# Microsoft/multiverso

Measured on AMD Instinct MI355X. Metric: MatrixTable Add+Get updates/sec (whole node), higher is better.
Workload: dtype fp32; 1 GPU; model=MatrixTable 1000000x128 dense sgd updater, global_batch=1, parallelism=ps-sharded dp1 (reduce-scatter/all-gather over xGMI)

## Files before the change

multiverso_amd/ops/csrc/bindings.cpp:

```cpp

#include <torch/extension.h>
#include <ATen/hip/HIPContext.h>
#include <cstdint>

extern "C" {
void mv_launch_copy(void*, const float*, int, int64_t, hipStream_t);
void mv_launch_add(float*, const void*, int, int64_t, hipStream_t, int);
void mv_launch_add_f64(double*, const double*, int64_t, hipStream_t, int);
void mv_launch_add_i32(int32_t*, const int32_t*, int64_t, hipStream_t, int);
void mv_launch_add_i64(int64_t*, const int64_t*, int64_t, hipStream_t, int);
void mv_launch_sgd(float*, const void*, void*, int, float, int64_t,
                   hipStream_t, int);
void mv_launch_sgd_f64(double*, const double*, double*, double, int64_t,
                       hipStream_t, int);
void mv_launch_momentum(float*, float*, const void*, void*, int, float,
                        int64_t, hipStream_t, int);
void mv_launch_momentum_f64(double*, double*, const double*, double, int64_t,
                            hipStream_t, int);
void mv_launch_adagrad(float*, float*, const void*, void*, int, float, float,
                       float, int64_t, hipStream_t, int);
void mv_launch_adagrad_f64(double*, double*, const double*, double, double,
                           double, int64_t, hipStream_t, int);
void mv_launch_dcasgd(float*, float*, const void*, void*, int, float, float,
                      int64_t, hipStream_t, int);
void mv_launch_dcasgda(float*, float*, float*, const void*, void*, int, float,
                       float, float, float, int64_t, hipStream_t, int);
void mv_launch_adam(float*, float*, float*, const void*, void*, int, double,
                    double, double, double, double, double, int64_t,
                    hipStream_t, int);
void mv_launch_adam_f64(double*, double*, double*, const double*, double,
                        double, double, double, double, double, int64_t,
                        hipStream_t, int);
void mv_launch_onebit_encode(const float*, float*, uint8_t*, int64_t,
                             hipStream_t);
void mv_launch_onebit_decode_sum(float*, const uint8_t*, int, int64_t,
                                 hipStream_t);
void mv_launch_row_gather(void*, int, const float*, const int64_t*, int64_t,
                          int64_t, hipStream_t);
void mv_launch_row_scatter_add(float*, const void*, int, const int64_t*, float,
                               int64_t, int64_t, int, hipStream_t);
void mv_launch_w2v(float*, float*, float*, float*, const int64_t*, const int*,
                   const int64_t*, const float*, const int*, float, int64_t,
                   int64_t, int, int, hipStream_t);
void mv_launch_w2v_ns(float*, float*, float*, float*, const int64_t*,
                      const int*, const int64_t*, const int64_t*, int64_t,
                      int, uint64_t, float, int64_t, int64_t, int, int,
                      hipStream_t);
void mv_launch_lr_sigmoid_fwd(const float*, const int64_t*, const float*,
                              const int*, const float*, const float*,
                              float*, float*, int64_t, hipStream_t);
void mv_launch_lr_sigmoid_scatter(float*, const int64_t*, const float*,
                                  const int*, const float*, float, int,
                                  float, int64_t, hipStream_t);
void mv_launch_row_scatter_adagrad(float*, float*, const void*, int,
                                   const int64_t*, float, float, float,
                                   int64_t, int64_t, int, hipStream_t);
void mv_launch_row_momentum(float*, float*, const void*, int, const int64_t*,
                            const int64_t*, float, int64_t, int64_t,
                            hipStream_t);
void mv_launch_row_dcasgd(float*, float*, const void*, int, const int64_t*,
                          const int64_t*, float, float, int64_t, int64_t,
                          hipStream_t);
void mv_launch_row_dcasgda(float*, float*, float*, const void*, int,
                           const int64_t*, const int64_t*, float, float,
                           float, float, int64_t, int64_t, hipStream_t);
void mv_launch_row_adam(float*, float*, float*, const void*, int,
                        const int64_t*, const int64_t*, double, double,
                        double, double, double, double, int64_t, int64_t,
                        hipStream_t);
void mv_launch_lr_softmax_fwd(const float*, const int64_t*, const float*,
                              const int*, const float*, const float*,
                              float*, float*, int64_t, int64_t, hipStream_t);
void mv_launch_lr_softmax_scatter(float*, const int64_t*, const float*,
                                  const int*, const float*, float, int,
                                  float, int64_t, int64_t, hipStream_t);
void mv_launch_lr_dense_post(float*, const float*, const float*, float*,
                             float, int64_t, int64_t, hipStream_t);
int mv_launch_lr_dense_fwd(const float*, const float*, const float*,
                           const float*, float*, float*, float, int64_t,
                           int64_t, int64_t, int, hipStream_t);
void mv_launch_lr_ftrl_fwd(const float*, const int64_t*, const float*,
                           const int*, const float*, const float*, float*,
                           float*, float, float, float, float, int64_t,
                           int64_t, hipStream_t);
void mv_launch_lr_ftrl_scatter(float*, const int64_t*, const float*,
                               const int*, const float*, float, float,
                               float, float, int64_t, int64_t, hipStream_t);
}

namespace {

hipStream_t cur_stream() {
  return at::hip::getCurrentHIPStream().stream();
}

void check_f32(const torch::Tensor& t, const char* name) {
  TORCH_CHECK(t.is_cuda(), name, " must be on GPU");
  TORCH_CHECK(t.is_contiguous(), name, " must be contiguous");
  TORCH_CHECK(t.scalar_type() == torch::kFloat32, name, " must be fp32");
}

void check_dev(const torch::Tensor& t, const char* name,
               torch::ScalarType st) {
  TORCH_CHECK(t.is_cuda(), name, " must be on GPU");
  TORCH_CHECK(t.is_contiguous(), name, " must be contiguous");
  TORCH_CHECK(t.scalar_type() == st, name, " dtype mismatch");
}

using Named = std::pair<const char*, torch::Tensor>;
int64_t check_same(std::initializer_list<Named> ts,
                   c10::optional<torch::ScalarType> st = c10::nullopt) {
  for (const auto& t : ts) {
    if (st) check_dev(t.second, t.first, *st);
    else check_f32(t.second, t.first);
  }
  int64_t n = ts.begin()->second.numel();
  for (const auto& t : ts)
    TORCH_CHECK(t.second.numel() == n, "size mismatch");
  return n;
}

float* f32(const torch::Tensor& t) { return t.data_ptr<float>(); }
double* f64(const torch::Tensor& t) { return t.data_ptr<double>(); }

constexpr int kWireDelta = 1, kWireOut = 2;

int wire_bit(const torch::Tensor& t, const char* name, int64_t n, int bit,
             c10::optional<torch::ScalarType> st = c10::nullopt) {
  TORCH_CHECK(t.is_cuda(), name, " must be on GPU");
  TORCH_CHECK(t.is_contiguous(), name, " must be contiguous");
  TORCH_CHECK(t.numel() == n, "size mismatch");
  auto want = st.value_or(torch::kFloat32);
  if (want == torch::kFloat32 && t.scalar_type() == torch::kBFloat16)
    return bit;
  if (st) {
    TORCH_CHECK(t.scalar_type() == want, name, " dtype mismatch");
  } else {
    TORCH_CHECK(t.scalar_type() == want, name, " must be fp32 or bf16");
  }
  return 0;
}

void nt_copy(torch::Tensor dst, torch::Tensor src) {
  int64_t n = check_same({{"src", src}});
  int wire = wire_bit(dst, "dst", n, kWireOut);
  mv_launch_copy(dst.data_ptr(), f32(src), wire, n, cur_stream());
}

void add_inplace(torch::Tensor data, torch::Tensor delta, bool reverse) {
  auto st = data.scalar_type();
  int64_t n = check_same({{"data", data}}, st);
  int wire = wire_bit(delta, "delta", n, kWireDelta, st);
  if (st == torch::kFloat32)
    mv_launch_add(f32(data), delta.data_ptr(), wire, n, cur_stream(), reverse);
  else if (st == torch::kFloat64)
    mv_launch_add_f64(f64(data), f64(delta), n, cur_stream(), reverse);
  else if (st == torch::kInt32)
    mv_launch_add_i32(data.data_ptr<int32_t>(), delta.data_ptr<int32_t>(), n,
// ... 420 lines not shown
  TORCH_CHECK(ptr.scalar_type() == torch::kInt32, "ptr must be int32");
  int64_t B = ptr.numel() - 1;
  TORCH_CHECK(err.numel() == B, "err size mismatch");
  mv_launch_lr_sigmoid_scatter(w.data_ptr<float>(), keys.data_ptr<int64_t>(),
                               vals.data_ptr<float>(), ptr.data_ptr<int>(),
                               err.data_ptr<float>(), (float)lr,
                               (int)reg_type, (float)reg_coef, B,
                               cur_stream());
}

void lr_softmax_forward(torch::Tensor w, torch::Tensor keys,
                        torch::Tensor vals, torch::Tensor ptr,
                        torch::Tensor labels,
                        c10::optional<torch::Tensor> wts,
                        torch::Tensor err, torch::Tensor loss, int64_t K) {
  check_f32(w, "w"); check_f32(vals, "vals"); check_f32(labels, "labels");
  check_f32(err, "err"); check_f32(loss, "loss");
  TORCH_CHECK(keys.scalar_type() == torch::kInt64, "keys must be int64");
  TORCH_CHECK(ptr.scalar_type() == torch::kInt32, "ptr must be int32");
  TORCH_CHECK(K >= 2 && K <= 64,
              "fused softmax supports 2..64 classes (got ", K, ")");
  int64_t B = ptr.numel() - 1;
  TORCH_CHECK(labels.numel() == B && loss.numel() == B, "batch mismatch");
  TORCH_CHECK(err.numel() == B * K, "err must be [B, K]");
  TORCH_CHECK(keys.numel() == vals.numel(), "keys/vals mismatch");
  const float* wp = nullptr;
  if (wts.has_value()) {
    check_f32(*wts, "wts");
    TORCH_CHECK(wts->numel() == B, "weights size mismatch");
    wp = wts->data_ptr<float>();
  }
  mv_launch_lr_softmax_fwd(w.data_ptr<float>(), keys.data_ptr<int64_t>(),
                           vals.data_ptr<float>(), ptr.data_ptr<int>(),
                           labels.data_ptr<float>(), wp,
                           err.data_ptr<float>(), loss.data_ptr<float>(),
                           B, K, cur_stream());
}

void lr_softmax_scatter(torch::Tensor w, torch::Tensor keys,
                        torch::Tensor vals, torch::Tensor ptr,
                        torch::Tensor err, double lr, int64_t reg_type,
                        double reg_coef, int64_t K) {
  check_f32(w, "w"); check_f32(vals, "vals"); check_f32(err, "err");
  TORCH_CHECK(keys.scalar_type() == torch::kInt64, "keys must be int64");
  TORCH_CHECK(ptr.scalar_type() == torch::kInt32, "ptr must be int32");
  int64_t B = ptr.numel() - 1;
  TORCH_CHECK(err.numel() == B * K, "err must be [B, K]");
  mv_launch_lr_softmax_scatter(w.data_ptr<float>(), keys.data_ptr<int64_t>(),
                               vals.data_ptr<float>(), ptr.data_ptr<int>(),
                               err.data_ptr<float>(), (float)lr,
                               (int)reg_type, (float)reg_coef, B, K,
                               cur_stream());
}

void lr_ftrl_forward(torch::Tensor zn, torch::Tensor keys,
                     torch::Tensor vals, torch::Tensor ptr,
                     torch::Tensor labels, c10::optional<torch::Tensor> wts,
                     torch::Tensor err, torch::Tensor loss, double alpha,
                     double beta, double l1, double l2, int64_t K) {
  check_f32(zn, "zn"); check_f32(vals, "vals"); check_f32(labels, "labels");
  check_f32(err, "err"); check_f32(loss, "loss");
  TORCH_CHECK(keys.scalar_type() == torch::kInt64, "keys must be int64");
  TORCH_CHECK(ptr.scalar_type() == torch::kInt32, "ptr must be int32");
  TORCH_CHECK(K >= 1 && K <= 32,
              "fused FTRL supports 1..32 outputs (got ", K, ")");
  int64_t B = ptr.numel() - 1;
  TORCH_CHECK(labels.numel() == B && loss.numel() == B, "batch mismatch");
  TORCH_CHECK(err.numel() == B * K, "err must be [B, K]");
  const float* wp = nullptr;
  if (wts.has_value()) {
    check_f32(*wts, "wts");
    wp = wts->data_ptr<float>();
  }
  mv_launch_lr_ftrl_fwd(zn.data_ptr<float>(), keys.data_ptr<int64_t>(),
                        vals.data_ptr<float>(), ptr.data_ptr<int>(),
                        labels.data_ptr<float>(), wp, err.data_ptr<float>(),
                        loss.data_ptr<float>(), (float)(1.0 / alpha),
                        (float)beta, (float)l1, (float)l2, B, K,
                        cur_stream());
}

void lr_dense_post(torch::Tensor logits, torch::Tensor labels,
                   c10::optional<torch::Tensor> wts, torch::Tensor loss_acc,
                   double inv_b) {
  check_f32(logits, "logits"); check_f32(labels, "labels");
  check_f32(loss_acc, "loss_acc");
  int64_t B = labels.numel();
  TORCH_CHECK(B > 0 && logits.numel() % B == 0,
              "logits/labels batch mismatch");
  int64_t K = logits.numel() / B;
  TORCH_CHECK(K >= 1 && K <= 64,
              "fused dense post supports 1..64 classes (got ", K, ")");
  TORCH_CHECK(loss_acc.numel() == 1, "loss_acc must be a scalar");
  const float* wp = nullptr;
  if (wts.has_value()) {
    check_f32(*wts, "wts");
    TORCH_CHECK(wts->numel() == B, "weights size mismatch");
    wp = wts->data_ptr<float>();
  }
  mv_launch_lr_dense_post(logits.data_ptr<float>(),
                          labels.data_ptr<float>(), wp,
                          loss_acc.data_ptr<float>(), (float)inv_b, B, K,
                          cur_stream());
}

bool lr_dense_fwd(torch::Tensor x, torch::Tensor w, torch::Tensor labels,
                  c10::optional<torch::Tensor> wts, torch::Tensor diff,
                  torch::Tensor loss_acc, double inv_b, bool nt) {
  check_f32(x, "x"); check_f32(w, "w"); check_f32(labels, "labels");
  check_f32(diff, "diff"); check_f32(loss_acc, "loss_acc");
  TORCH_CHECK(x.dim() == 2 && w.dim() == 2 && x.size(1) == w.size(0),
              "x [B,d] and w [d,K] shape mismatch");
  TORCH_CHECK(x.is_contiguous() && w.is_contiguous(), "x/w must be "
              "contiguous");
  int64_t B = x.size(0), d = x.size(1), K = w.size(1);
  TORCH_CHECK(labels.numel() == B, "labels batch mismatch");
  TORCH_CHECK(diff.numel() == B * K, "diff must be [B, K]");
  TORCH_CHECK(loss_acc.numel() == 1, "loss_acc must be a scalar");
  const float* wp = nullptr;
  if (wts.has_value()) {
    check_f32(*wts, "wts");
    TORCH_CHECK(wts->numel() == B, "weights size mismatch");
    wp = wts->data_ptr<float>();
  }
  return mv_launch_lr_dense_fwd(
             x.data_ptr<float>(), w.data_ptr<float>(),
             labels.data_ptr<float>(), wp, diff.data_ptr<float>(),
             loss_acc.data_ptr<float>(), (float)inv_b, B, d, K,
             nt ? 1 : 0, cur_stream()) != 0;
}


void lr_ftrl_scatter(torch::Tensor zn, torch::Tensor keys,
                     torch::Tensor vals, torch::Tensor ptr,
                     torch::Tensor err, double alpha, double beta, double l1,
                     double l2, int64_t K) {
  check_f32(zn, "zn"); check_f32(vals, "vals"); check_f32(err, "err");
  TORCH_CHECK(keys.scalar_type() == torch::kInt64, "keys must be int64");
  TORCH_CHECK(ptr.scalar_type() == torch::kInt32, "ptr must be int32");
  int64_t B = ptr.numel() - 1;
  TORCH_CHECK(err.numel() == B * K, "err must be [B, K]");
  mv_launch_lr_ftrl_scatter(zn.data_ptr<float>(), keys.data_ptr<int64_t>(),
                            vals.data_ptr<float>(), ptr.data_ptr<int>(),
                            err.data_ptr<float>(), (float)(1.0 / alpha),
                            (float)beta, (float)l1, (float)l2, B, K,
                            cur_stream());
}

}

PYBIND11_MODULE(TORCH_EXTENSION_NAME, m) {
  auto rev = py::arg("reverse") = false;
  auto data = py::arg("data"), delta = py::arg("delta"), out = py::arg("out");
  m.def("add_inplace", &add_inplace, "K1: data += delta (fp32, fused)", data,
        delta, rev);
  m.def("nt_copy", &nt_copy,
        "K7: non-temporal streaming copy (a bf16 dst narrows)");
  m.def("sgd_update", &sgd_update, "K2: data -= delta", data, delta, rev);
  m.def("momentum_update", &momentum_update, "K3: fused momentum update",
        data, py::arg("m"), delta, py::arg("mu"), rev);
  m.def("adagrad_update", &adagrad_update, "K4: fused adagrad update", data,
        py::arg("gsq"), delta, py::arg("lr"), py::arg("rho"), py::arg("eps"),
        rev);
  m.def("momentum_copy_update", &momentum_copy_update,
        "fused momentum Add+Get", data, py::arg("m"), delta, out,
        py::arg("mu"), rev);
  m.def("adagrad_copy_update", &adagrad_copy_update,
        "fused adagrad Add+Get", data, py::arg("gsq"), delta, out,
        py::arg("lr"), py::arg("rho"), py::arg("eps"), rev);
  m.def("dcasgd_copy_update", &dcasgd_copy_update,
        "fused dcasgd Add+Get", data, py::arg("bak"), delta, out,
        py::arg("lr"), py::arg("lambda_"), rev);
  m.def("dcasgda_copy_update", &dcasgda_copy_update,
        "fused dcasgda Add+Get", data, py::arg("bak"), py::arg("msq"), delta,
        out, py::arg("lr"), py::arg("lambda_"), py::arg("rho"),
        py::arg("eps"), rev);
  m.def("sgd_copy_update", &sgd_copy_update,
        "fused Add+Get: data (+/-)= delta; out = data (saves the Get's "
        "shard re-read at N=1)", data, delta, out, py::arg("sign"), rev);
  m.def("dcasgd_update", &dcasgd_update,
        "DC-ASGD: delay-compensated update with per-worker backup", data,
        py::arg("bak"), delta, py::arg("lr"), py::arg("lambda_"), rev);
  m.def("dcasgda_update", &dcasgda_update,
        "DC-ASGD-a: adaptive lambda via mean-square of gradients", data,
        py::arg("bak"), py::arg("msq"), delta, py::arg("lr"),
        py::arg("lambda_"), py::arg("rho"), py::arg("eps"), rev);
  m.def("adam_update", &adam_update,
        "fused Adam/AdamW step (fp32, fp64); step = lr/(1-b1^t), "
        "rbc2 = 1/sqrt(1-b2^t), decay = 1-lr*wd",
        py::arg("data"), py::arg("m"), py::arg("v"), py::arg("delta"),
        py::arg("b1"), py::arg("b2"), py::arg("step"), py::arg("rbc2"),
        py::arg("decay"), py::arg("eps"), rev);
  m.def("adam_copy_update", &adam_copy_update, "fused adam Add+Get",
        py::arg("data"), py::arg("m"), py::arg("v"), py::arg("delta"),
        py::arg("out"), py::arg("b1"), py::arg("b2"), py::arg("step"),
        py::arg("rbc2"), py::arg("decay"), py::arg("eps"), rev);
  m.def("onebit_encode", &onebit_encode,
        "1-bit wire: payload = code(residual + delta), residual = the error",
        py::arg("delta"), py::arg("residual"), py::arg("payload"));
  m.def("onebit_decode_sum", &onebit_decode_sum,
        "1-bit wire: out = sum over nparts payloads of their decoded values",
        py::arg("out"), py::arg("payloads"), py::arg("nparts"));
  m.def("row_gather", &row_gather,
        "K6: out[i] = shard[rows[i]]; dtype=torch.bfloat16 narrows",
        py::arg("shard"), py::arg("rows"), py::arg("dtype") = py::none());
  m.def("row_gather_out", &row_gather_out, "K6 (preallocated out)");
  m.def("row_scatter_add", &row_scatter_add,
        "K5: shard[rows[i]] += sign*vals[i] (atomic; assume_unique=True "
        "uses plain stores)", py::arg("shard"), py::arg("rows"),
        py::arg("vals"), py::arg("sign"), py::arg("assume_unique") = false);
  m.def("lr_sigmoid_forward", &lr_sigmoid_forward,
        "K13 fused: per-sample CSR dot + sigmoid + error/loss");
  m.def("lr_sigmoid_scatter", &lr_sigmoid_scatter,
        "K14 fused: w[keys] -= lr*(vals*err + reg), atomic");
  m.def("lr_softmax_forward", &lr_softmax_forward,
        "K13 softmax fused: per-sample CSR K-class logits + softmax + "
        "err/loss (objective.cpp:193-230)");
  m.def("lr_softmax_scatter", &lr_softmax_scatter,
        "K14 softmax fused: w[key*K+k] -= lr*(val*err_k + reg), atomic");
  m.def("lr_dense_fwd", &lr_dense_fwd,
        "Dense-mode fused forward: X@W + softmax/sigmoid diff + loss in "
        "one kernel, W LDS-staged; returns False when d*K exceeds the "
        "LDS budget (caller uses the GEMM + lr_dense_post path)",
        py::arg("x"), py::arg("w"), py::arg("labels"), py::arg("wts"),
        py::arg("diff"), py::arg("loss_acc"), py::arg("inv_b"),
        py::arg("nt") = true);
  m.def("lr_dense_post", &lr_dense_post,
        "Dense-mode fused post-GEMM: logits -> softmax/sigmoid diff in "
        "place + atomic mean-loss accumulate (objective.cpp:193-230 "
        "dense branch)");
  m.def("lr_ftrl_forward", &lr_ftrl_forward,
        "FTRL fused forward: reconstruct w from (z|n), sigmoid, err/loss "
        "(objective.cpp:250-345)");
  m.def("lr_ftrl_scatter", &lr_ftrl_scatter,
        "FTRL fused z/n state update (updater.cpp:79-101 applied to the "
        "local chunk buffer)");
  m.def("row_scatter_adagrad", &row_scatter_adagrad,
        "K15: keyed adagrad update on owned shard rows "
        "(assume_unique=True uses plain stores)",
        py::arg("shard"), py::arg("gsq"), py::arg("rows"), py::arg("vals"),
        py::arg("lr"), py::arg("rho"), py::arg("eps"),
        py::arg("assume_unique") = false);
  m.def("row_momentum_update", &row_momentum_update,
        "keyed momentum: sum value rows per row id (equal ids adjacent in "
        "rows; perm maps list position to vals row), one step per row",
        py::arg("shard"), py::arg("m"), py::arg("rows"), py::arg("vals"),
        py::arg("mu"), py::arg("perm") = py::none());
  m.def("row_dcasgd_update", &row_dcasgd_update,
        "keyed DC-ASGD, same row/perm contract as row_momentum_update",
        py::arg("shard"), py::arg("bak"), py::arg("rows"), py::arg("vals"),
        py::arg("lr"), py::arg("lam"), py::arg("perm") = py::none());
  m.def("row_dcasgda_update", &row_dcasgda_update,
        "keyed DC-ASGD-a, same row/perm contract as row_momentum_update",
        py::arg("shard"), py::arg("bak"), py::arg("msq"), py::arg("rows"),
        py::arg("vals"), py::arg("lr"), py::arg("lam"), py::arg("rho"),
        py::arg("eps"), py::arg("perm") = py::none());
  m.def("row_adam_update", &row_adam_update,
        "keyed Adam, same row/perm contract as row_momentum_update",
        py::arg("shard"), py::arg("m"), py::arg("v"), py::arg("rows"),
        py::arg("vals"), py::arg("b1"), py::arg("b2"), py::arg("step"),
        py::arg("rbc2"), py::arg("decay"), py::arg("eps"),
        py::arg("perm") = py::none());
  m.def("w2v_train", &w2v_train,
        "K9-K11: fused word2vec block training (skip-gram/CBOW, NS/HS, "
        "optional adagrad)");
  m.def("w2v_train_ns", &w2v_train_ns,
        "K9-K11 NS fast path: negatives generated in-kernel from the "
        "per-block pool (reference LCG scheme)");
}
```

multiverso_amd/ops/csrc/kernels.hip:

```cpp

#include <hip/hip_runtime.h>
#include <cstdint>
#include <cstdio>
#include <cstdlib>
#include <type_traits>

#define WAVE 64
#define BLOCK 256
#define MAX_GRID 2048
#define ELEM_GRID 1024
#define STATE_GRID 768
#define UPD_GRID 768
#define COPY_BLOCK 1024

typedef float v4f __attribute__((ext_vector_type(4)));

static __device__ __forceinline__ v4f ntload(const v4f* p) {
  return __builtin_nontemporal_load(p);
}
static __device__ __forceinline__ void ntstore(v4f* p, v4f v) {
  __builtin_nontemporal_store(v, p);
}
template <class T>
static __device__ __forceinline__ T ntload(const T* p) { return *p; }
template <class T>
static __device__ __forceinline__ void ntstore(T* p, T v) { *p = v; }

static __device__ __forceinline__ float rsq(float x) {
  return __frsqrt_rn(x);
}
static __device__ __forceinline__ v4f rsq(v4f x) {
  v4f r;
  r.x = __frsqrt_rn(x.x); r.y = __frsqrt_rn(x.y);
  r.z = __frsqrt_rn(x.z); r.w = __frsqrt_rn(x.w);
  return r;
}

template <class V, class T>
static __device__ __forceinline__ V ld(const T* p, int64_t i) {
  return ntload((const V*)p + i);
}
template <class V, class T>
static __device__ __forceinline__ void st(T* p, int64_t i, V v) {
  ntstore((V*)p + i, v);
}

template <class V, bool KEEP, class T>
static __device__ __forceinline__ V ld_shard(const T* p, int64_t i) {
  if constexpr (KEEP) return *((const V*)p + i);
  else return ld<V>(p, i);
}

struct bf16 { uint16_t bits; };
typedef uint16_t v4h __attribute__((ext_vector_type(4)));
typedef uint16_t v2h __attribute__((ext_vector_type(2)));

static __device__ __forceinline__ float widen(uint16_t h) {
  return __builtin_bit_cast(float, (uint32_t)h << 16);
}
static __device__ __forceinline__ uint16_t narrow(float f) {
  return __builtin_bit_cast(uint16_t, (__bf16)f);
}

template <class V>
static __device__ __forceinline__ V ld(const bf16* p, int64_t i) {
  if constexpr (std::is_same<V, v4f>::value) {
    v4h h = __builtin_nontemporal_load((const v4h*)p + i);
    v4f v;
    v.x = widen(h.x); v.y = widen(h.y); v.z = widen(h.z); v.w = widen(h.w);
    return v;
  } else {
    static_assert(std::is_same<V, float>::value, "bf16 widens to fp32");
    return widen(p[i].bits);
  }
}
template <class V>
static __device__ __forceinline__ void st(bf16* p, int64_t i, V v) {
  if constexpr (sizeof(V) == 16) {
    v4h h;
    h.x = narrow(v.x); h.y = narrow(v.y); h.z = narrow(v.z); h.w = narrow(v.w);
    if constexpr (std::is_same<V, v4f>::value)
      __builtin_nontemporal_store(h, (v4h*)p + i);
    else
      *((v4h*)p + i) = h;
  } else if constexpr (sizeof(V) == 8) {
    v2h h;
    h.x = narrow(v.x); h.y = narrow(v.y);
    *((v2h*)p + i) = h;
  } else {
    p[i].bits = narrow(v);
  }
}

#define WIRE_DELTA 1
#define WIRE_OUT 2
#define ELEM_OF(p) std::remove_cv_t<std::remove_pointer_t<decltype(p)>>

template <class F>
static void with_wire(int wire, const void* delta, void* out, F f) {
  switch (wire & (WIRE_DELTA | WIRE_OUT)) {
    case 0: f((const float*)delta, (float*)out); break;
    case WIRE_DELTA: f((const bf16*)delta, (float*)out); break;
    case WIRE_OUT: f((const float*)delta, (bf16*)out); break;
    default: f((const bf16*)delta, (bf16*)out);
  }
}

static inline bool vec_ok(const float*) { return true; }
static inline bool vec_ok(const bf16* p) { return ((uintptr_t)p & 7) == 0; }

static inline int grid_for_cap(int64_t work_items, int cap,
                               int block = BLOCK) {
  int64_t blocks = (work_items + block - 1) / block;
  if (blocks > cap) blocks = cap;
  if (blocks < 1) blocks = 1;
  return (int)blocks;
}
static inline int grid_for(int64_t work_items) {
  return grid_for_cap(work_items, MAX_GRID);
}


template <class T, class D = T>
struct AddOp {
  using elem = T;
  T* data; const D* delta;
  template <class V> __device__ __forceinline__ V step(int64_t i) const {
    V v = ld_shard<V, true>(data, i) + ld<V>(delta, i);
    st(data, i, v);
    return v;
  }
};

template <class T, class D = T>
struct SgdOp {
  using elem = T;
  T* data; const D* delta; T sign;
  template <class V> __device__ __forceinline__ V step(int64_t i) const {
    V v = ld_shard<V, true>(data, i) + sign * ld<V>(delta, i);
    st(data, i, v);
    return v;
  }
};

template <class T, class D = T>
struct MomentumOp {
  using elem = T;
  T* data; T* m; const D* delta; T mu;
  template <class V, bool KEEP = false>
  __device__ __forceinline__ V step_at(int64_t i, V g) const {
    V d = ld_shard<V, KEEP>(data, i);
    V mm = __builtin_elementwise_fma((V)mu, ld<V>(m, i), ((T)1 - mu) * g);
    st(m, i, mm);
    d -= mm;
    st(data, i, d);
    return d;
  }
  template <class V> __device__ __forceinline__ V step(int64_t i) const {
    return step_at<V, true>(i, ld<V>(delta, i));
  }
};

template <class T, class D = T>
struct AdagradOp {
  using elem = T;
  T* data; T* gsq; const D* delta; T inv_lr, rho, eps;
  template <class V> __device__ __forceinline__ V step(int64_t i) const {
    V d = ld_shard<V, true>(data, i), G = ld<V>(gsq, i);
    V g = ld<V>(delta, i) * inv_lr;
    G += g * g;
    if constexpr (std::is_same<T, double>::value) d -= rho * g / sqrt(G + eps);
    else d -= rho * g * rsq(G + eps);
    st(gsq, i, G);
    st(data, i, d);
    return d;
  }
};

template <class D = float>
struct DcasgdOp {
  using elem = float;
  float* data; float* bak; const D* delta; float lr, lambda;
  template <class V, bool KEEP = false>
  __device__ __forceinline__ V step_at(int64_t i, V g) const {
    V w = ld_shard<V, KEEP>(data, i), b = ld<V>(bak, i);
    w -= lr * (g + lambda * g * g * (w - b));
    st(data, i, w);
    st(bak, i, w);
    return w;
  }
  template <class V> __device__ __forceinline__ V step(int64_t i) const {
    return step_at<V, true>(i, ld<V>(delta, i));
  }
};

template <class D = float>
struct DcasgdaOp {
  using elem = float;
  float* data; float* bak; float* msq; const D* delta;
  float lr, lambda, rho, eps;
  template <class V, bool KEEP = false>
  __device__ __forceinline__ V step_at(int64_t i, V g) const {
    V w = ld_shard<V, KEEP>(data, i), b = ld<V>(bak, i);
    V m = rho * ld<V>(msq, i) + (1.0f - rho) * g * g;
    st(msq, i, m);
    V lam = lambda * rsq(m + eps);
    w -= lr * (g + lam * g * g * (w - b));
    st(data, i, w);
    st(bak, i, w);
    return w;
  }
  template <class V> __device__ __forceinline__ V step(int64_t i) const {
    return step_at<V, true>(i, ld<V>(delta, i));
  }
};

template <class T, class D = T>
struct AdamOp {
  using elem = T;
  T* data; T* m; T* v; const D* delta;
  T b1, omb1, b2, omb2, alpha, rbc2, decay, eps;
  template <class V, bool KEEP = false>
  __device__ __forceinline__ V step_at(int64_t i, V g) const {
    V w = ld_shard<V, KEEP>(data, i), mm = ld<V>(m, i), vv = ld<V>(v, i);
    mm = __builtin_elementwise_fma((V)b1, mm, omb1 * g);
    vv = __builtin_elementwise_fma((V)b2, vv, omb2 * g * g);
    V den = __builtin_elementwise_fma(__builtin_elementwise_sqrt(vv), (V)rbc2,
                                      (V)eps);
    w = __builtin_elementwise_fma((V)(-alpha), mm / den, w * decay);
    st(m, i, mm);
    st(v, i, vv);
    st(data, i, w);
    return w;
  }
  template <class V> __device__ __forceinline__ V step(int64_t i) const {
    return step_at<V, true>(i, ld<V>(delta, i));
  }
};

template <class T, class D>
static AdamOp<T, D> adam_op(T* data, T* m, T* v, const D* delta, double b1,
                            double b2, double step, double rbc2, double decay,
                            double eps) {
  return AdamOp<T, D>{data, m, v, delta, (T)b1, (T)(1.0 - b1), (T)b2,
                      (T)(1.0 - b2), (T)step, (T)rbc2, (T)decay, (T)eps};
}

template <class O = float>
struct CopyOp {
  using elem = float;
  O* dst; const float* src;
  template <class V> __device__ __forceinline__ V step(int64_t i) const {
    V v = ld<V>(src, i);
    st(dst, i, v);
    return v;
  }
};

template <class Op, class V, bool COPY, class O>
__global__ void k_elem(Op op, O* __restrict__ out, int64_t start, int64_t n,
                       int rev) {
  int64_t stride = (int64_t)gridDim.x * blockDim.x;
  int64_t n_pad = (n + (WAVE - 1)) & ~(int64_t)(WAVE - 1);
  for (int64_t i = start + (int64_t)blockIdx.x * blockDim.x + threadIdx.x;
       i < n_pad; i += stride) {
    int64_t lane = threadIdx.x & (WAVE - 1);
    int64_t j = rev ? n_pad - WAVE - i + 2 * lane : i;
    if (j < n) {
      V v = op.template step<V>(j);
      if (COPY) st(out, j, v);
    }
  }
}

template <bool COPY, class Op, class O>
static void launch_elem(const Op& op, O* out, int64_t n, int cap, int block,
                        hipStream_t s, bool vec = true, int rev = 0) {
  using T = typename Op::elem;
  if constexpr (std::is_same<T, float>::value) {
    if (vec) {
      int64_t n4 = n / 4;
      if (n4) k_elem<Op, v4f, COPY><<<grid_for_cap(n4, cap, block), block, 0,
                                      s>>>(op, out, 0, n4, rev);
      if (n > n4 * 4) k_elem<Op, float, COPY><<<1, 64, 0, s>>>(op, out,
                                                               n4 * 4, n, 0);
      return;
    }
  }
  if (n > 0)
    k_elem<Op, T, COPY><<<grid_for_cap(n, cap, block), block, 0, s>>>(
        op, out, 0, n, rev);
}

template <class Op, class O>
static void launch_update(const Op& op, O* out, int64_t n, int cap,
                          hipStream_t s, int rev) {
  bool vec = vec_ok(op.delta) && vec_ok(out);
  if (out) launch_elem<true>(op, out, n, cap, BLOCK, s, vec, rev);
  else launch_elem<false>(op, (float*)nullptr, n, cap, BLOCK, s, vec, rev);
}

extern "C" {

void mv_launch_copy(void* dst, const float* src, int wire, int64_t n,
                    hipStream_t s) {
  with_wire(wire, nullptr, dst, [&](auto*, auto* o) {
    launch_elem<false>(CopyOp<ELEM_OF(o)>{o, src}, (float*)nullptr, n,
                       ELEM_GRID, BLOCK, s, vec_ok(o));
  });
}

void mv_launch_add(float* data, const void* delta, int wire, int64_t n,
                   hipStream_t s, int rev) {
  with_wire(wire, delta, nullptr, [&](auto* d, auto*) {
    launch_elem<false>(AddOp<float, ELEM_OF(d)>{data, d}, (float*)nullptr, n,
                       UPD_GRID, BLOCK, s, vec_ok(d), rev);
  });
}
void mv_launch_add_f64(double* d, const double* x, int64_t n, hipStream_t s,
                       int rev) {
  launch_elem<false>(AddOp<double>{d, x}, (double*)nullptr, n, ELEM_GRID,
                     BLOCK, s, true, rev);
}
void mv_launch_add_i32(int32_t* d, const int32_t* x, int64_t n, hipStream_t s,
                       int rev) {
  launch_elem<false>(AddOp<int32_t>{d, x}, (int32_t*)nullptr, n, ELEM_GRID,
                     BLOCK, s, true, rev);
}
void mv_launch_add_i64(int64_t* d, const int64_t* x, int64_t n, hipStream_t s,
                       int rev) {
  launch_elem<false>(AddOp<int64_t>{d, x}, (int64_t*)nullptr, n, ELEM_GRID,
                     BLOCK, s, true, rev);
}

void mv_launch_sgd(float* data, const void* delta, void* out, int wire,
                   float sign, int64_t n, hipStream_t s, int rev) {
  with_wire(wire, delta, out, [&](auto* d, auto* o) {
    launch_update(SgdOp<float, ELEM_OF(d)>{data, d, sign}, o, n, UPD_GRID, s,
                  rev);
  });
}
void mv_launch_sgd_f64(double* d, const double* x, double* out, double sign,
                       int64_t n, hipStream_t s, int rev) {
  SgdOp<double> op{d, x, sign};
  if (out) launch_elem<true>(op, out, n, STATE_GRID, BLOCK, s, true, rev);
  else launch_elem<false>(op, out, n, ELEM_GRID, BLOCK, s, true, rev);
}

void mv_launch_momentum(float* data, float* m, const void* delta, void* out,
                        int wire, float mu, int64_t n, hipStream_t s, int rev) {
  with_wire(wire, delta, out, [&](auto* d, auto* o) {
    launch_update(MomentumOp<float, ELEM_OF(d)>{data, m, d, mu}, o, n,
                  STATE_GRID, s, rev);
  });
}
void mv_launch_momentum_f64(double* d, double* m, const double* x, double mu,
                            int64_t n, hipStream_t s, int rev) {
  launch_elem<false>(MomentumOp<double>{d, m, x, mu}, (double*)nullptr, n,
                     STATE_GRID, BLOCK, s, true, rev);
}

void mv_launch_adagrad(float* data, float* gsq, const void* delta, void* out,
                       int wire, float lr, float rho, float eps, int64_t n,
                       hipStream_t s, int rev) {
  with_wire(wire, delta, out, [&](auto* d, auto* o) {
    launch_update(AdagradOp<float, ELEM_OF(d)>{data, gsq, d, 1.0f / lr, rho,
                                               eps},
                  o, n, STATE_GRID, s, rev);
  });
}
void mv_launch_adagrad_f64(double* d, double* g, const double* x, double lr,
                           double rho, double eps, int64_t n, hipStream_t s,
                           int rev) {
  launch_elem<false>(AdagradOp<double>{d, g, x, 1.0 / lr, rho, eps},
                     (double*)nullptr, n, STATE_GRID, BLOCK, s, true, rev);
}

void mv_launch_dcasgd(float* data, float* bak, const void* delta, void* out,
                      int wire, float lr, float lambda, int64_t n,
                      hipStream_t s, int rev) {
  with_wire(wire, delta, out, [&](auto* d, auto* o) {
    launch_update(DcasgdOp<ELEM_OF(d)>{data, bak, d, lr, lambda}, o, n,
                  STATE_GRID, s, rev);
  });
}

void mv_launch_dcasgda(float* data, float* bak, float* msq, const void* delta,
                       void* out, int wire, float lr, float lambda, float rho,
                       float eps, int64_t n, hipStream_t s, int rev) {
  with_wire(wire, delta, out, [&](auto* d, auto* o) {
    launch_update(DcasgdaOp<ELEM_OF(d)>{data, bak, msq, d, lr, lambda, rho,
                                        eps},
                  o, n, STATE_GRID, s, rev);
  });
}

void mv_launch_adam(float* data, float* m, float* v, const void* delta,
                    void* out, int wire, double b1, double b2, double step,
                    double rbc2, double decay, double eps, int64_t n,
                    hipStream_t s, int rev) {
  with_wire(wire, delta, out, [&](auto* d, auto* o) {
    launch_update(adam_op(data, m, v, d, b1, b2, step, rbc2, decay, eps), o,
                  n, STATE_GRID, s, rev);
  });
}
void mv_launch_adam_f64(double* d, double* m, double* v, const double* x,
                        double b1, double b2, double step, double rbc2,
                        double decay, double eps, int64_t n, hipStream_t s,
                        int rev) {
  launch_elem<false>(adam_op(d, m, v, x, b1, b2, step, rbc2, decay, eps),
                     (double*)nullptr, n, STATE_GRID, BLOCK, s, true, rev);
}

}


template <class V, class O, class Idx>
__global__ void k_row_gather(O* __restrict__ out, const V* __restrict__ shard,
                             const int64_t* __restrict__ rows,
                             Idx total, Idx cols) {
  Idx stride = (Idx)gridDim.x * blockDim.x;
  for (Idx i = (Idx)blockIdx.x * blockDim.x + threadIdx.x; i < total;
       i += stride) {
    Idx r = i / cols, c = i - r * cols;
    V v = shard[rows[r] * (int64_t)cols + c];
    if constexpr (std::is_same<O, bf16>::value) st(out, i, v);
    else ((V*)out)[i] = v;
  }
}

template <class D, class Idx, bool ATOMIC>
__global__ void k_row_scatter_add(float* __restrict__ shard,
                                  const D* __restrict__ vals,
                                  const int64_t* __restrict__ rows,
                                  float sign, Idx total, Idx cols) {
  Idx stride = (Idx)gridDim.x * blockDim.x;
  for (Idx i = (Idx)blockIdx.x * blockDim.x + threadIdx.x; i < total;
       i += stride) {
    Idx r = i / cols, c = i - r * cols;
    int64_t k = rows[r] * (int64_t)cols + c;
    float x = ld<float>(vals, i);
    if (ATOMIC) atomicAdd(&shard[k], sign * x);
    else shard[k] += sign * x;
  }
}

template <class D, class Idx, bool ATOMIC>
__global__ void k_row_scatter_adagrad(float* __restrict__ shard,
                                      float* __restrict__ gsq,
                                      const D* __restrict__ vals,
                                      const int64_t* __restrict__ rows,
                                      float inv_lr, float rho, float eps,
                                      Idx total, Idx cols) {
  Idx stride = (Idx)gridDim.x * blockDim.x;
  for (Idx i = (Idx)blockIdx.x * blockDim.x + threadIdx.x; i < total;
       i += stride) {
    Idx r = i / cols, c = i - r * cols;
    int64_t k = rows[r] * (int64_t)cols + c;
    float g = ld<float>(vals, i) * inv_lr;
    if (g != 0.0f) {
      float G;
      if (ATOMIC) G = atomicAdd(&gsq[k], g * g) + g * g;
      else { G = gsq[k] + g * g; gsq[k] = G; }
      float dw = -rho * g * rsq(G + eps);
      if (ATOMIC) atomicAdd(&shard[k], dw);
      else shard[k] += dw;
    }
  }
}

template <class Op, class V, class Idx, class D>
__global__ void k_row_update(Op op, const D* __restrict__ vals,
                             const int64_t* __restrict__ rows,
                             const int64_t* __restrict__ perm, int64_t n,
                             Idx total, Idx cols) {
  Idx stride = (Idx)gridDim.x * blockDim.x;
  for (Idx i = (Idx)blockIdx.x * blockDim.x + threadIdx.x; i < total;
       i += stride) {
    Idx j = i / cols, c = i - j * cols;
    int64_t r = rows[j];
    if (j > 0 && rows[j - 1] == r) continue;
    int64_t k = j;
    V sum = ld<V>(vals, (perm ? perm[k] : k) * (int64_t)cols + c);
    for (++k; k < n && rows[k] == r; ++k)
      sum += ld<V>(vals, (perm ? perm[k] : k) * (int64_t)cols + c);
    op.template step_at<V>(r * (int64_t)cols + c, sum);
  }
}

static inline bool aligned16(const void* p) {
  return ((uintptr_t)p & 15) == 0;
}
// ... 1021 lines not shown
```

Before: 445.1 billion updates/s.

## Use atomic ticket-based dynamic chunk scheduling in fp32 updater kernels

```diff
diff --git a/multiverso_amd/ops/csrc/bindings.cpp b/multiverso_amd/ops/csrc/bindings.cpp
--- a/multiverso_amd/ops/csrc/bindings.cpp
+++ b/multiverso_amd/ops/csrc/bindings.cpp
@@ -4,6 +4,8 @@
 #include <cstdint>
 
 extern "C" {
+int64_t mv_elem_chunk();
+int mv_elem_grid_cap();
 void mv_launch_copy(void*, const float*, int, int64_t, hipStream_t);
 void mv_launch_add(float*, const void*, int, int64_t, hipStream_t, int);
 void mv_launch_add_f64(double*, const double*, int64_t, hipStream_t, int);
@@ -730,6 +732,10 @@
 PYBIND11_MODULE(TORCH_EXTENSION_NAME, m) {
   auto rev = py::arg("reverse") = false;
   auto data = py::arg("data"), delta = py::arg("delta"), out = py::arg("out");
+  m.def("elem_chunk", &mv_elem_chunk,
+        "float4 vectors per ticket chunk of the fp32 updater kernels");
+  m.def("elem_grid_cap", &mv_elem_grid_cap,
+        "grid cap (blocks) of the fp32 updater kernels");
   m.def("add_inplace", &add_inplace, "K1: data += delta (fp32, fused)", data,
         delta, rev);
   m.def("nt_copy", &nt_copy,
diff --git a/multiverso_amd/ops/csrc/kernels.hip b/multiverso_amd/ops/csrc/kernels.hip
--- a/multiverso_amd/ops/csrc/kernels.hip
+++ b/multiverso_amd/ops/csrc/kernels.hip
@@ -3,15 +3,20 @@
 #include <cstdint>
 #include <cstdio>
 #include <cstdlib>
+#include <mutex>
 #include <type_traits>
 
 #define WAVE 64
 #define BLOCK 256
 #define MAX_GRID 2048
 #define ELEM_GRID 1024
+#define TICKET_GRID 512
 #define STATE_GRID 768
 #define UPD_GRID 768
 #define COPY_BLOCK 1024
+
+#define TICKET_U 8
+#define TICKET_SLOTS 64
 
 typedef float v4f __attribute__((ext_vector_type(4)));
 
@@ -259,7 +264,29 @@
 
 template <class Op, class V, bool COPY, class O>
 __global__ void k_elem(Op op, O* __restrict__ out, int64_t start, int64_t n,
-                       int rev) {
+                       int rev, unsigned long long* ticket) {
+  if (ticket) {
+    __shared__ int64_t s_t[2];
+    const int64_t chunk = (int64_t)TICKET_U * blockDim.x;
+    const int64_t nchunks = (n + chunk - 1) / chunk;
+    if (threadIdx.x == 0) s_t[0] = (int64_t)atomicAdd(ticket, 1ULL);
+    __syncthreads();
+    int p = 0;
+    for (int64_t t = s_t[0]; t < nchunks; t = s_t[p]) {
+      int64_t j = (rev ? nchunks - 1 - t : t) * chunk + threadIdx.x;
+#pragma unroll
+      for (int u = 0; u < TICKET_U; ++u, j += blockDim.x) {
+        if (j < n) {
+          V v = op.template step<V>(j);
+          if (COPY) st(out, j, v);
+        }
+      }
+      if (threadIdx.x == 0) s_t[p ^ 1] = (int64_t)atomicAdd(ticket, 1ULL);
+      __syncthreads();
+      p ^= 1;
+    }
+    return;
+  }
   int64_t stride = (int64_t)gridDim.x * blockDim.x;
   int64_t n_pad = (n + (WAVE - 1)) & ~(int64_t)(WAVE - 1);
   for (int64_t i = start + (int64_t)blockIdx.x * blockDim.x + threadIdx.x;
@@ -273,34 +300,96 @@
   }
 }
 
+struct alignas(128) TicketLine { unsigned long long next; };
+__device__ TicketLine g_tickets[TICKET_SLOTS];
+
+static void ticket_lost(const char* why) {
+  static std::once_flag once;
+  std::call_once(once, [&] {
+    fprintf(stderr, "multiverso_amd: no ticket counter for an updater launch "
+                    "(%s); it and its like run the static loop\n", why);
+  });
+}
+
+static unsigned long long* ticket_for(hipStream_t s) {
+  constexpr int MAX_DEV = 64;
+  static std::mutex mu;
+  static TicketLine* base[MAX_DEV];
+  static hipStream_t owner[MAX_DEV][TICKET_SLOTS];
+  static int used[MAX_DEV];
+  int dev = 0;
+  if (s == hipStreamPerThread) {
+    ticket_lost("hipStreamPerThread is not one stream");
+    return nullptr;
+  }
+  if (hipGetDevice(&dev) != hipSuccess || dev < 0 || dev >= MAX_DEV) {
+    ticket_lost("no current device below 64");
+    return nullptr;
+  }
+  std::lock_guard<std::mutex> lock(mu);
+  if (!base[dev]) {
+    void* p = nullptr;
+    hipError_t e = hipGetSymbolAddress(&p, HIP_SYMBOL(g_tickets));
+    if (e != hipSuccess) {
+      ticket_lost(hipGetErrorString(e));
+      return nullptr;
+    }
+    base[dev] = (TicketLine*)p;
+  }
+  for (int k = 0; k < used[dev]; ++k)
+    if (owner[dev][k] == s) return &base[dev][k].next;
+  if (used[dev] == TICKET_SLOTS) {
+    ticket_lost("all counters of the device are taken");
+    return nullptr;
+  }
+  owner[dev][used[dev]] = s;
+  return &base[dev][used[dev]++].next;
+}
+
 template <bool COPY, class Op, class O>
 static void launch_elem(const Op& op, O* out, int64_t n, int cap, int block,
-                        hipStream_t s, bool vec = true, int rev = 0) {
+                        hipStream_t s, bool vec = true, int rev = 0,
+                        bool tickets = false) {
   using T = typename Op::elem;
   if constexpr (std::is_same<T, float>::value) {
     if (vec) {
       int64_t n4 = n / 4;
-      if (n4) k_elem<Op, v4f, COPY><<<grid_for_cap(n4, cap, block), block, 0,
-                                      s>>>(op, out, 0, n4, rev);
-      if (n > n4 * 4) k_elem<Op, float, COPY><<<1, 64, 0, s>>>(op, out,
-                                                               n4 * 4, n, 0);
+      unsigned long long* ticket = tickets && n4 ? ticket_for(s) : nullptr;
+      if (ticket) {
+        hipError_t e = hipMemsetAsync(ticket, 0, sizeof *ticket, s);
+        if (e != hipSuccess) {
+          ticket_lost(hipGetErrorString(e));
+          ticket = nullptr;
+        }
+      }
+      int grid = ticket ? grid_for_cap((n4 + TICKET_U - 1) / TICKET_U,
+                                       TICKET_GRID, block)
+                        : grid_for_cap(n4, cap, block);
+      if (n4) k_elem<Op, v4f, COPY><<<grid, block, 0, s>>>(op, out, 0, n4,
+                                                           rev, ticket);
+      if (n > n4 * 4) k_elem<Op, float, COPY><<<1, 64, 0, s>>>(
+          op, out, n4 * 4, n, 0, nullptr);
       return;
     }
   }
   if (n > 0)
     k_elem<Op, T, COPY><<<grid_for_cap(n, cap, block), block, 0, s>>>(
-        op, out, 0, n, rev);
+        op, out, 0, n, rev, nullptr);
 }
 
 template <class Op, class O>
 static void launch_update(const Op& op, O* out, int64_t n, int cap,
-                          hipStream_t s, int rev) {
+                          hipStream_t s, int rev, bool unfused_tickets = true) {
   bool vec = vec_ok(op.delta) && vec_ok(out);
-  if (out) launch_elem<true>(op, out, n, cap, BLOCK, s, vec, rev);
-  else launch_elem<false>(op, (float*)nullptr, n, cap, BLOCK, s, vec, rev);
+  if (out) launch_elem<true>(op, out, n, cap, BLOCK, s, vec, rev, true);
+  else launch_elem<false>(op, (float*)nullptr, n, cap, BLOCK, s, vec, rev,
+                          unfused_tickets);
 }
 
 extern "C" {
+
+int64_t mv_elem_chunk() { return (int64_t)TICKET_U * BLOCK; }
+int mv_elem_grid_cap() { return TICKET_GRID; }
 
 void mv_launch_copy(void* dst, const float* src, int wire, int64_t n,
                     hipStream_t s) {
@@ -337,7 +426,7 @@
                    float sign, int64_t n, hipStream_t s, int rev) {
   with_wire(wire, delta, out, [&](auto* d, auto* o) {
     launch_update(SgdOp<float, ELEM_OF(d)>{data, d, sign}, o, n, UPD_GRID, s,
-                  rev);
+                  rev, false);
   });
 }
 void mv_launch_sgd_f64(double* d, const double* x, double* out, double sign,
```

New measurement: 444.8 billion updates/s. Within noise of the previous version (-0.1%).
